# bridgedp/hunter_bipedal_control

Measured on NVIDIA H100. Metric: MPC+WBC control-step solves/sec (Hunter N=100), higher is better.
Workload: dtype f64

## Files before the change

hunter_bipedal_control_b200/csrc/hb_api.cu:

```cuda
#include <cuda_runtime.h>
#include <math.h>
#include <stdio.h>
#include <stdlib.h>
#include <string.h>

#include <new>

#include "../../include/hunter_b200.h"
#include "hb_common.cuh"
#include "hb_mpc.cuh"
#include "hb_planner.h"
#include <algorithm>
#include <string>
#include <utility>
#include <atomic>
#include <mutex>
#include <cstring>
#include <thread>
#include <vector>
#include "hb_qp.cuh"
#include "hb_rbd.cuh"
#include "hb_sqp.cuh"
#include "hb_wbc.cuh"
#include "hb_hoqp.cuh"
#include "hb_rollout.cuh"
#include "hb_estimator.cuh"
#include "hb_trajectory.cuh"
#include "hb_reference.cuh"

using namespace hb;

template <class T> struct InstanceSetting {
  T* dev;
  int n;
  std::vector<T> host;
  const T* get() const { return n > 0 ? dev : nullptr; }
};

struct hb_ctx {
  hb_config cfg;
  hb_wbc_settings wbc;
  int32_t wbc_form;
  int device;
  cudaStream_t stream;
  cudaStream_t stream_main, stream_aux;
  int base;
  int64_t launches;
  double *dxt, *dut, *perf;
  void* sqp_mem; double *lin, *proj, *rk;
  int32_t* flags;
  double *xdes, *udes;
  int32_t *wstatus, *witers, *wmode;
  void* hoqp_mem; double* hoqp_scratch;
  double *cyc_xref, *cyc_swing, *cyc_tk;
  int32_t *cyc_mode, *cyc_nn;
  double *res_t0, *res_xt, *res_ut, *res_tk;
  int32_t *res_mode, *res_nn;
  int res_valid;
  double* res_sol; int res_sol_valid;
  double* res_stance;
  void* ro_mem;
  hb_rollout_command* ro_cmd; hb_plan_input* ro_in; hb_reference* ro_refs; hb_solve_info* ro_info; int32_t* ro_pstat;
  double *ro_t0, *ro_x0, *ro_feet, *ro_sol, *ro_jcmd, *ro_jtau, *ro_tau, *ro_held, *ro_tnow, *ro_wrench;
  void* re_mem;
  double *re_quat, *re_gyro, *re_acc, *re_jpos, *re_jvel, *re_rbd;
  uint8_t* re_flag;
  InstanceSetting<hb_push_schedule> pushes;
  InstanceSetting<hb_plant_variation> variations;
  InstanceSetting<hb_terrain> terrains;
  void* arena; size_t arena_cap;
  void* pinned; size_t pinned_cap;
  int last_cuda;
  size_t last_h2d_bytes;
  int prof_on, prof_n;
  cudaEvent_t* prof_ev;
  int* prof_kind;
};

namespace {

enum { HB_OK = 0, HB_EINVAL = -1, HB_ECUDA = -2, HB_ENOMEM = -3, HB_ECAP = -4, HB_EPLAN = -5, HB_ECOMM = -6 };

#define CK(call)                                   \
  do {                                             \
    cudaError_t e__ = (call);                      \
    if (e__ != cudaSuccess) { if (ctx) ctx->last_cuda = (int)e__; return HB_ECUDA; } \
  } while (0)

constexpr int PROF_MAX = 4096;
enum { K_UNPROFILED = -1, K_BACKWARD = 0, K_FORWARD_LS = 1, K_WBC_ASSEMBLE = 2, K_QP = 3, K_OTHER = 4, K_LIN = 5, K_LQ = 6, K_NKINDS = 7 };

template <class T> cudaError_t dalloc(T** p, size_t n) { return cudaMalloc(reinterpret_cast<void**>(p), n * sizeof(T)); }

inline void prof_begin(hb_ctx* ctx, int kind) {
  if (ctx->prof_on && ctx->prof_n < PROF_MAX) { ctx->prof_kind[ctx->prof_n] = kind; cudaEventRecord(ctx->prof_ev[2 * ctx->prof_n], ctx->stream); }
}
inline void prof_end(hb_ctx* ctx) {
  if (ctx->prof_on && ctx->prof_n < PROF_MAX) { cudaEventRecord(ctx->prof_ev[2 * ctx->prof_n + 1], ctx->stream); ctx->prof_n++; }
}

template <class... P, class... A>
int launch(hb_ctx* ctx, int kind, void (*kernel)(P...), dim3 grid, dim3 block, size_t smem, A&&... args) {
  if (kind != K_UNPROFILED) prof_begin(ctx, kind);
  kernel<<<grid, block, smem, ctx->stream>>>(std::forward<A>(args)...);
  if (kind != K_UNPROFILED) prof_end(ctx);
  ctx->launches++;
  CK(cudaGetLastError());
  return HB_OK;
}

int set_device(hb_ctx* ctx) { return cudaSetDevice(ctx->device) == cudaSuccess ? HB_OK : HB_ECUDA; }

enum Cap : bool { UNCAPPED = false, CAPPED = true };
constexpr int EMPTY = 1;
inline bool no_host_check() { return true; }
template <class F = bool (*)()> int enter(hb_ctx* ctx, int B, bool args, Cap cap, const F& host_ok = no_host_check) {
  if (!ctx || B < 0 || !args) return HB_EINVAL;
  if (B == 0) return EMPTY;
  if (cap && ctx->base + B > ctx->cfg.max_batch) return HB_ECAP;
  if (!host_ok()) return HB_EINVAL;
  return set_device(ctx);
}
#define ENTER(...)                                                   \
  do {                                                               \
    const int rc__ = enter(__VA_ARGS__);                             \
    if (rc__) return rc__ == EMPTY ? HB_OK : rc__;                   \
  } while (0)

template <class T> bool all_ok(int B, const T* src, bool (*ok)(const T&)) {
  if (src) for (int i = 0; i < B; ++i) if (!ok(src[i])) return false;
  return true;
}
// ... 147 lines not shown
    case HB_ENOMEM: return "out of memory";
    case HB_ECAP: return "batch exceeds context capacity";
    case HB_EPLAN: return "reference planner: swing phase without take-off / touch-down time, or reference capacity exceeded";
    case HB_ECOMM: return "NCCL not available or a collective failed (hb_shard_last_error)";
    default: return "unknown error";
  }
}

int hb_create(const hb_config* cfg, int device, hb_ctx** out) {
  if (!cfg || !out || cfg->horizon_N < 1 || cfg->horizon_N > HB_MAX_HORIZON || cfg->max_batch < 1 || !(cfg->dt > 0.0) || cfg->time_horizon < 0.0) return HB_EINVAL;
  hb_ctx* ctx = new (std::nothrow) hb_ctx();
  if (!ctx) return HB_ENOMEM;
  memset(ctx, 0, sizeof(*ctx));
  ctx->cfg = *cfg;
  ctx->device = device;
  hb_default_wbc_settings(&ctx->wbc);
  if (cudaSetDevice(device) != cudaSuccess) { hb_destroy(ctx); return HB_ECUDA; }
  if (cudaStreamCreateWithFlags(&ctx->stream, cudaStreamNonBlocking) != cudaSuccess) { ctx->stream = nullptr; hb_destroy(ctx); return HB_ECUDA; }
  ctx->stream_main = ctx->stream;
  if (cudaStreamCreateWithFlags(&ctx->stream_aux, cudaStreamNonBlocking) != cudaSuccess) { ctx->stream_aux = nullptr; hb_destroy(ctx); return HB_ECUDA; }
  Model* m = new Model();
  memset(m, 0, sizeof(Model));
  for (int b = 0; b < NBODY; ++b) {
    for (int i = 0; i < 3; ++i) { m->joint_xyz[3 * b + i] = HB_JOINT_XYZ[3 * b + i]; m->com[3 * b + i] = HB_BODY_COM[3 * b + i]; }
    for (int i = 0; i < 9; ++i) m->inertia[9 * b + i] = HB_BODY_INERTIA[9 * b + i];
    m->mass[b] = HB_BODY_MASS[b];
    int code = 0;
    for (int i = 0; i < 3; ++i) if (HB_JOINT_AXIS[3 * b + i] != 0.0) code = (HB_JOINT_AXIS[3 * b + i] > 0 ? 1 : -1) * (i + 1);
    m->joint_axis[b] = code;
  }
  m->total_mass = HB_TOTAL_MASS;
  for (int i = 0; i < 12; ++i) m->contact_offset[i] = HB_CONTACT_OFFSET[i];
  for (int j = 0; j < NJ; ++j) { m->joint_lower[j] = HB_JOINT_LOWER[j]; m->joint_upper[j] = HB_JOINT_UPPER[j]; m->joint_vel_limit[j] = HB_JOINT_VEL_LIMIT[j]; m->torque_limit[j] = HB_WBC_TORQUE_LIMITS[j % 5]; }
  for (int i = 0; i < NX; ++i) m->Q[i] = HB_Q_DIAG[i];
  cudaError_t e = cudaMemcpyToSymbol(c_model, m, sizeof(Model));
  if (e == cudaSuccess) {
    double* dR = nullptr;
    e = dalloc(&dR, NU * NU);
    if (e == cudaSuccess) {
      init_input_cost_kernel<<<1, 32, 0, ctx->stream>>>(dR);
      e = cudaStreamSynchronize(ctx->stream);
      if (e == cudaSuccess) e = cudaMemcpy(m->R, dR, sizeof(double) * NU * NU, cudaMemcpyDeviceToHost);
      if (e == cudaSuccess) e = cudaMemcpyToSymbol(c_model, m, sizeof(Model));
      cudaFree(dR);
    }
  }
  if (e == cudaSuccess) {
    double tab[32 * LQ_LANE_TAB] = {};
    for (int l = 0; l < 32; ++l) {
      double* t = tab + l * LQ_LANE_TAB;
      if (l < NX) t[0] = m->Q[l];
      if (l < 12) t[1] = m->R[l * NU + l];
      if (l >= 12 && l < NU) for (int j = 0; j < NJ; ++j) t[2 + j] = m->R[l * NU + 12 + j];
      if (l < 10) { t[12] = m->joint_lower[l]; t[13] = m->joint_upper[l]; }
      else if (l < 20) { t[12] = -m->joint_vel_limit[l - 10]; t[13] = m->joint_vel_limit[l - 10]; }
    }
    e = cudaMemcpyToSymbol(g_lq_lane, tab, sizeof(tab));
  }
  delete m;
  if (e != cudaSuccess) { ctx->last_cuda = (int)e; hb_destroy(ctx); return HB_ECUDA; }
  const size_t B = cfg->max_batch, N = cfg->horizon_N;
  bool ok = true;
  ok = ok && dalloc(&ctx->dxt, B * (N + 1) * NX) == cudaSuccess && dalloc(&ctx->dut, B * N * NU) == cudaSuccess;
  ok = ok && dalloc(&ctx->perf, B * 4) == cudaSuccess && dalloc(&ctx->flags, B) == cudaSuccess;
  ok = ok && dalloc(&ctx->xdes, B * NX) == cudaSuccess && dalloc(&ctx->udes, B * NU) == cudaSuccess;
  ok = ok && dalloc(&ctx->wstatus, B) == cudaSuccess && dalloc(&ctx->witers, B) == cudaSuccess && dalloc(&ctx->wmode, B) == cudaSuccess;
  ok = ok && dalloc(&ctx->cyc_xref, B * (N + 1) * NX) == cudaSuccess && dalloc(&ctx->cyc_swing, B * (N + 1) * 24) == cudaSuccess;
  ok = ok && dalloc(&ctx->cyc_mode, B * (N + 1)) == cudaSuccess && dalloc(&ctx->cyc_tk, B * (N + 1)) == cudaSuccess && dalloc(&ctx->cyc_nn, B) == cudaSuccess;
  ok = ok && dalloc(&ctx->res_xt, B * (N + 1) * NX) == cudaSuccess && dalloc(&ctx->res_ut, B * N * NU) == cudaSuccess && dalloc(&ctx->res_t0, B) == cudaSuccess;
  ok = ok && dalloc(&ctx->res_mode, B * (N + 1)) == cudaSuccess && dalloc(&ctx->res_tk, B * (N + 1)) == cudaSuccess && dalloc(&ctx->res_nn, B) == cudaSuccess;
  ok = ok && dalloc(&ctx->res_sol, B * NWBC) == cudaSuccess && dalloc(&ctx->res_stance, B * 12) == cudaSuccess;
  if (!ok) { hb_destroy(ctx); return HB_ENOMEM; }
  {
    cudaError_t fe = cudaSuccess;
    auto attr = [&](const void* fn, size_t bytes) { if (fe == cudaSuccess) fe = cudaFuncSetAttribute(fn, cudaFuncAttributeMaxDynamicSharedMemorySize, (int)bytes); };
    attr((const void*)probe_flow_map_kernel, sizeof(ProbeShared));
    attr((const void*)qp_batch_kernel, 200 * 1024);
    attr((const void*)wbc_fused_kernel, wbc_fused_doubles() * sizeof(double));
    attr((const void*)hoqp_kernel, hoqp_smem_bytes());
    attr((const void*)hwbc_fused_kernel, hwbc_fused_bytes());
    attr((const void*)lin_kernel, 4 * sizeof(LinHalf) + sizeof(ChainModel));
    attr((const void*)lq_kernel, sizeof(LqShared));
    attr((const void*)riccati_kernel, sizeof(RicShared));
    attr((const void*)forward_linesearch2_kernel, sizeof(Fw2Shared));
    attr((const void*)warm_shift_kernel, sizeof(double) * ((N + 1) * NX + N * NU));
    for (const void* fn : {(const void*)wbc_fused_kernel, (const void*)riccati_kernel, (const void*)lq_kernel, (const void*)hwbc_fused_kernel})
      if (fe == cudaSuccess) fe = cudaFuncSetAttribute(fn, cudaFuncAttributePreferredSharedMemoryCarveout, (int)cudaSharedmemCarveoutMaxShared);
    if (fe != cudaSuccess) { ctx->last_cuda = (int)fe; hb_destroy(ctx); return HB_ECUDA; }
  }
  *out = ctx;
  return HB_OK;
}

int hb_destroy(hb_ctx* ctx) {
  if (!ctx) return HB_EINVAL;
  cudaSetDevice(ctx->device);
  void* ptrs[] = {ctx->sqp_mem, ctx->dxt, ctx->dut, ctx->perf, ctx->flags, ctx->xdes, ctx->udes, ctx->wstatus, ctx->witers, ctx->wmode,
                  ctx->hoqp_mem, ctx->cyc_xref, ctx->cyc_swing, ctx->cyc_tk, ctx->cyc_mode, ctx->cyc_nn, ctx->res_t0, ctx->res_xt,
                  ctx->res_ut, ctx->res_tk, ctx->res_mode, ctx->res_nn, ctx->res_sol, ctx->res_stance, ctx->arena, ctx->ro_mem, ctx->re_mem,
                  ctx->pushes.dev, ctx->variations.dev, ctx->terrains.dev};
  for (void* p : ptrs) if (p) cudaFree(p);
  if (ctx->pinned) cudaFreeHost(ctx->pinned);
  if (ctx->prof_ev) { for (int i = 0; i < 2 * PROF_MAX; ++i) cudaEventDestroy(ctx->prof_ev[i]); delete[] ctx->prof_ev; delete[] ctx->prof_kind; }
  if (ctx->stream_aux) cudaStreamDestroy(ctx->stream_aux);
  if (ctx->stream_main) cudaStreamDestroy(ctx->stream_main);
  else if (ctx->stream) cudaStreamDestroy(ctx->stream);
  delete ctx;
  return HB_OK;
}

int hb_sync(hb_ctx* ctx) {
  if (!ctx) return HB_EINVAL;
  CK(cudaStreamSynchronize(ctx->stream));
  return HB_OK;
}
int hb_profile_enable(hb_ctx* ctx, int on) {
  if (!ctx) return HB_EINVAL;
  if (set_device(ctx)) return HB_ECUDA;
  if (on && !ctx->prof_ev) {
    ctx->prof_ev = new (std::nothrow) cudaEvent_t[2 * PROF_MAX];
    ctx->prof_kind = new (std::nothrow) int[PROF_MAX];
    if (!ctx->prof_ev || !ctx->prof_kind) return HB_ENOMEM;
    for (int i = 0; i < 2 * PROF_MAX; ++i) CK(cudaEventCreate(&ctx->prof_ev[i]));
  }
  ctx->prof_on = on ? 1 : 0;
  ctx->prof_n = 0;
  return HB_OK;
}

int hb_profile_read(hb_ctx* ctx, double* ms_per_kind, int64_t* count_per_kind) {
  if (!ctx || !ms_per_kind || !count_per_kind) return HB_EINVAL;
  if (set_device(ctx)) return HB_ECUDA;
  CK(cudaStreamSynchronize(ctx->stream));
  for (int k = 0; k < K_NKINDS; ++k) { ms_per_kind[k] = 0.0; count_per_kind[k] = 0; }
  for (int i = 0; i < ctx->prof_n; ++i) {
    float ms = 0.f;
    CK(cudaEventElapsedTime(&ms, ctx->prof_ev[2 * i], ctx->prof_ev[2 * i + 1]));
    ms_per_kind[ctx->prof_kind[i]] += ms;
    count_per_kind[ctx->prof_kind[i]]++;
  }
  ctx->prof_n = 0;
  return HB_OK;
}

const char* hb_last_cuda_error(const hb_ctx* ctx) { return ctx ? cudaGetErrorString((cudaError_t)ctx->last_cuda) : "no context"; }

int64_t hb_launch_count(const hb_ctx* ctx) { return ctx ? ctx->launches : 0; }
int64_t hb_last_reference_upload_bytes(const hb_ctx* ctx) { return ctx ? (int64_t)ctx->last_h2d_bytes : 0; }
void* hb_stream(hb_ctx* ctx) { return ctx ? (void*)ctx->stream : nullptr; }

static int launch_qp(hb_ctx* ctx, int B, int n, int m, const double* H, const double* g, const double* A, const double* lbA, const double* ubA,
                     size_t sH, size_t sA, size_t sB, const int32_t* m_per, double* x, int32_t* status, int32_t* iters) {
  if (!qp_shape_ok(n, m)) return HB_EINVAL;
  const size_t per_warp = qp_workspace_doubles(n) * sizeof(double);
  int wpb = (int)((200 * 1024) / per_warp);
  if (wpb < 1) return HB_EINVAL;
  if (wpb > 1) wpb = 1;
  const int blocks = (B + wpb - 1) / wpb;
  return launch(ctx, K_QP, qp_batch_kernel, blocks, 32 * wpb, per_warp * wpb, B, n, m, H, g, A, lbA, ubA, sH, sA, sB, m_per, ctx->cfg.wbc_rho,
                ctx->cfg.qp_max_iter, x, status, iters);
}

int hb_wbc_qp_batch_dev(hb_ctx* ctx, int B, int n, int m, const double* H, const double* g, const double* A, const double* lbA,
                        const double* ubA, double* x, int32_t* status, int32_t* iters) {
  ENTER(ctx, B, H && g && A && lbA && ubA && x, UNCAPPED);
  return launch_qp(ctx, B, n, m, H, g, A, lbA, ubA, (size_t)n * n, (size_t)m * n, (size_t)m, nullptr, x, status, iters);
}

int hb_wbc_solve_batch_dev(hb_ctx* ctx, int B, const double* x_des, const double* u_des, const double* rbd, const int32_t* mode,
                           const uint8_t* stance_mode, double* sol, int32_t* status) {
  ENTER(ctx, B, x_des && u_des && rbd && mode && sol, CAPPED);
  return launch(ctx, K_QP, wbc_fused_kernel, B, 32, wbc_fused_doubles() * sizeof(double), B, ctx->wbc, x_des, u_des, rbd, mode, stance_mode,
                ctx->cfg.wbc_rho, ctx->cfg.qp_max_iter, sol, status ? status : ctx->wstatus + ctx->base, ctx->witers + ctx->base);
}

int hb_wbc_assemble_batch_dev(hb_ctx* ctx, int B, const double* x_des, const double* u_des, const double* rbd, const int32_t* mode,
                              const uint8_t* stance_mode, double* H, double* g, double* A, double* lbA, double* ubA, int32_t* m_rows) {
  ENTER(ctx, B, x_des && u_des && rbd && mode && H && g && A && lbA && ubA && m_rows, UNCAPPED);
  const int wpb = 4;
  return launch(ctx, K_WBC_ASSEMBLE, wbc_assemble_kernel, (B + wpb - 1) / wpb, 32 * wpb, sizeof(WbcShared) * wpb, B, ctx->wbc, x_des, u_des, rbd, mode,
                stance_mode, H, g, A, lbA, ubA, m_rows);
}

int hb_wbc_qp_rows_batch_dev(hb_ctx* ctx, int B, int n, int m_alloc, const int32_t* m_rows, const double* H, const double* g, const double* A,
                             const double* lbA, const double* ubA, double* x, int32_t* status, int32_t* iters) {
  ENTER(ctx, B, m_rows && H && g && A && lbA && ubA && x, UNCAPPED);
  return launch_qp(ctx, B, n, m_alloc, H, g, A, lbA, ubA, (size_t)n * n, (size_t)m_alloc * n, (size_t)m_alloc, m_rows, x, status, iters);
}

static int hoqp_reserve(hb_ctx* ctx) {
  const size_t Bc = ctx->cfg.max_batch;
  return reserve_group(&ctx->hoqp_mem, [&](void* m) {
    size_t off = 0;
    ctx->hoqp_scratch = carve<double>(m, off, Bc * HQ_SCRATCH);
    return off;
  });
}

int hb_hoqp_solve_batch_dev(hb_ctx* ctx, int B, const hb_hoqp_problem* problems, double* x, double* slack, int32_t* status) {
  ENTER(ctx, B, problems && x, CAPPED);
  const int rc = hoqp_reserve(ctx);
  if (rc) return rc;
  return launch(ctx, K_QP, hoqp_kernel, B, 32, hoqp_smem_bytes(), B, problems, ctx->hoqp_scratch, 2 * ctx->cfg.qp_max_iter, x, slack, status);
}

static int hwbc_tasks_dev(hb_ctx* ctx, int B, const double* x_des, const double* u_des, const double* rbd, const int32_t* mode, hb_hoqp_problem* problems) {
  return launch(ctx, K_WBC_ASSEMBLE, hwbc_tasks_kernel, B, 32, 0, B, ctx->wbc, x_des, u_des, rbd, mode, problems);
}

int hb_hierarchical_wbc_solve_batch_dev(hb_ctx* ctx, int B, const double* x_des, const double* u_des, const double* rbd, const int32_t* mode, double* sol,
                                        int32_t* status) {
  ENTER(ctx, B, x_des && u_des && rbd && mode && sol, CAPPED);
  return launch(ctx, K_QP, hwbc_fused_kernel, B, 32, hwbc_fused_bytes(), B, ctx->wbc, x_des, u_des, rbd, mode, 2 * ctx->cfg.qp_max_iter, sol, status);
}

static int controller_wbc_dev(hb_ctx* ctx, int B, const double* x_des, const double* u_des, const double* rbd, const int32_t* mode,
                              const uint8_t* stance_mode, double* sol, int32_t* status) {
  if (ctx->wbc_form == HB_WBC_HIERARCHICAL)
    return hb_hierarchical_wbc_solve_batch_dev(ctx, B, x_des, u_des, rbd, mode, sol, status ? status : ctx->wstatus + ctx->base);
  return hb_wbc_solve_batch_dev(ctx, B, x_des, u_des, rbd, mode, stance_mode, sol, status);
}

int hb_mpc_cold_start_batch_dev(hb_ctx* ctx, int B, const double* x0, const int32_t* mode, double* x_traj, double* u_traj) {
  ENTER(ctx, B, x0 && mode && x_traj && u_traj, UNCAPPED);
  return launch(ctx, K_UNPROFILED, cold_start_kernel, B, 128, 0, B, ctx->cfg.horizon_N, x0, mode, x_traj, u_traj);
}

static int mpc_solve_impl(hb_ctx* ctx, int B, const double* x0, const double* x_ref, const double* swing_ref, const int32_t* mode,
                          double* x_traj, double* u_traj, hb_solve_info* info, const double* tk, const int32_t* nn) {
  ENTER(ctx, B, x0 && x_ref && swing_ref && mode && x_traj && u_traj && (tk == nullptr) == (nn == nullptr), CAPPED);
  const size_t Bc = ctx->cfg.max_batch, Nc = ctx->cfg.horizon_N;
  int rc = reserve_group(&ctx->sqp_mem, [&](void* m) {
    size_t off = 0;
    ctx->lin = carve<double>(m, off, Bc * Nc * LIN_STRIDE); ctx->proj = carve<double>(m, off, Bc * Nc * PJ_STRIDE);
    ctx->rk = carve<double>(m, off, Bc * Nc * RK_STRIDE);
    return off;
  });
  if (rc) return rc;
  SqpArgs a;
  a.tk = tk; a.nn = nn;
  a.B = B; a.N = ctx->cfg.horizon_N; a.dt = ctx->cfg.dt; a.x_ref = x_ref; a.swing = swing_ref; a.mode = mode; a.xt = x_traj; a.ut = u_traj;
  {
    const size_t o = (size_t)ctx->base, Nn = (size_t)ctx->cfg.horizon_N;
    a.lin = ctx->lin + o * Nn * LIN_STRIDE; a.proj = ctx->proj + o * Nn * PJ_STRIDE; a.rk = ctx->rk + o * Nn * RK_STRIDE;
    a.dxt = ctx->dxt + o * (Nn + 1) * NX; a.dut = ctx->dut + o * Nn * NU; a.perf = ctx->perf + o * 4; a.flags = ctx->flags + o; a.x0 = x0;
  }
  const int N = a.N, NP = (N + 1) / 2;
  const long long nw = (long long)B * NP;
  rc = launch(ctx, K_LIN, lin_kernel, (unsigned)((nw + 1) / 2), 64, 4 * sizeof(LinHalf) + sizeof(ChainModel), a);
  if (!rc) rc = launch(ctx, K_LQ, lq_kernel, (unsigned)((long long)B * N), 32, sizeof(LqShared), a);
  if (!rc) rc = launch(ctx, K_BACKWARD, riccati_kernel, B, 64, sizeof(RicShared), a);
  if (!rc) rc = launch(ctx, K_FORWARD_LS, forward_linesearch2_kernel, B, 32, sizeof(Fw2Shared), a, ctx->cfg.line_search_max_trials, info);
  return rc;
}

int hb_mpc_solve_batch_dev(hb_ctx* ctx, int B, const double* x0, const double* x_ref, const double* swing_ref, const int32_t* mode,
                           double* x_traj, double* u_traj, hb_solve_info* info) {
  return mpc_solve_impl(ctx, B, x0, x_ref, swing_ref, mode, x_traj, u_traj, info, nullptr, nullptr);
}

int hb_mpc_solve_grid_batch_dev(hb_ctx* ctx, int B, const double* x0, const double* node_times, const int32_t* n_intervals, const double* x_ref,
                                const double* swing_ref, const int32_t* mode, double* x_traj, double* u_traj, hb_solve_info* info) {
  if (!node_times || !n_intervals) return HB_EINVAL;
  return mpc_solve_impl(ctx, B, x0, x_ref, swing_ref, mode, x_traj, u_traj, info, node_times, n_intervals);
}

static int policy_eval_impl(hb_ctx* ctx, int B, double t_rel, const double* x_traj, const double* u_traj, const int32_t* mode, double* x_des,
                            double* u_des, int32_t* mode_out, const double* tk, const int32_t* nn) {
  ENTER(ctx, B, x_traj && u_traj && mode && x_des && u_des && (tk == nullptr) == (nn == nullptr), UNCAPPED);
  const int wpb = 4;
  return launch(ctx, K_UNPROFILED, policy_eval_kernel, (B + wpb - 1) / wpb, 32 * wpb, 0, B, ctx->cfg.horizon_N, ctx->cfg.dt, t_rel, x_traj, u_traj, mode,
                x_des, u_des, mode_out, tk, nn, nullptr, nullptr);
}

int hb_policy_eval_batch_dev(hb_ctx* ctx, int B, double t_rel, const double* x_traj, const double* u_traj, const int32_t* mode, double* x_des,
                             double* u_des, int32_t* mode_out) {
  return policy_eval_impl(ctx, B, t_rel, x_traj, u_traj, mode, x_des, u_des, mode_out, nullptr, nullptr);
}

int hb_policy_eval_grid_batch_dev(hb_ctx* ctx, int B, double t_rel, const double* node_times, const int32_t* n_intervals, const double* x_traj,
                                  const double* u_traj, const int32_t* mode, double* x_des, double* u_des, int32_t* mode_out) {
  if (!node_times || !n_intervals) return HB_EINVAL;
  return policy_eval_impl(ctx, B, t_rel, x_traj, u_traj, mode, x_des, u_des, mode_out, node_times, n_intervals);
}

int hb_time_grid_batch_dev(hb_ctx* ctx, int B, const double* t0, const hb_reference* refs, double* node_times, int32_t* n_intervals, int32_t* status) {
  ENTER(ctx, B, t0 && refs && node_times && n_intervals, UNCAPPED);
  const double T = ctx->cfg.time_horizon > 0.0 ? ctx->cfg.time_horizon : ctx->cfg.horizon_N * ctx->cfg.dt;
  return launch(ctx, K_UNPROFILED, time_grid_kernel, (B + 127) / 128, 128, 0, B, ctx->cfg.horizon_N, ctx->cfg.dt, T, t0, refs, node_times, n_intervals, status);
}

static int control_step_impl(hb_ctx* ctx, int B, double t_rel, const double* x0, const double* x_ref, const double* swing_ref, const int32_t* mode,
                             const double* rbd, double* x_traj, double* u_traj, hb_solve_info* info, double* wbc_sol, double* torque,
                             int32_t* wbc_status, const double* tk, const int32_t* nn) {
  ENTER(ctx, B, x0 && x_ref && swing_ref && mode && rbd && x_traj && u_traj && wbc_sol && (tk == nullptr) == (nn == nullptr), CAPPED);
  int rc = mpc_solve_impl(ctx, B, x0, x_ref, swing_ref, mode, x_traj, u_traj, info, tk, nn);
  if (rc) return rc;
  double* xdes = ctx->xdes + (size_t)ctx->base * NX; double* udes = ctx->udes + (size_t)ctx->base * NU; int32_t* wmode = ctx->wmode + ctx->base;
  rc = policy_eval_impl(ctx, B, t_rel, x_traj, u_traj, mode, xdes, udes, wmode, tk, nn);
  if (rc) return rc;
  rc = controller_wbc_dev(ctx, B, xdes, udes, rbd, wmode, nullptr, wbc_sol, wbc_status);
  if (!rc && torque) rc = launch(ctx, K_UNPROFILED, torque_kernel, (B * NJ + 127) / 128, 128, 0, B, wbc_sol, torque);
  return rc;
}

int hb_control_step_batch_dev(hb_ctx* ctx, int B, double t_rel, const double* x0, const double* x_ref, const double* swing_ref, const int32_t* mode,
                              const double* rbd, double* x_traj, double* u_traj, hb_solve_info* info, double* wbc_sol, double* torque,
                              int32_t* wbc_status) {
  return control_step_impl(ctx, B, t_rel, x0, x_ref, swing_ref, mode, rbd, x_traj, u_traj, info, wbc_sol, torque, wbc_status, nullptr, nullptr);
}

static int wbc_fallback(hb_ctx* ctx, int B, bool no_prev, const int32_t* wbc_status, double* wbc_sol, double* torque) {
  if (!wbc_status) return HB_OK;
  const int have_prev = (!no_prev && ctx->res_sol_valid >= ctx->base + B) ? 1 : 0;
  const int rc = launch(ctx, K_UNPROFILED, wbc_fallback_kernel, (B * NWBC + 127) / 128, 128, 0, B, have_prev, wbc_status, wbc_sol,
                        ctx->res_sol + (size_t)ctx->base * NWBC, torque);
  if (rc) return rc;
  if (ctx->res_sol_valid < ctx->base + B) ctx->res_sol_valid = ctx->base + B;
  return HB_OK;
}

static int resident_cycle_impl(hb_ctx* ctx, int B, int cold_start, double t_rel, const double* t0, const double* x0, const hb_reference* refs,
                               const double* rbd, hb_solve_info* info, double* wbc_sol, double* torque, int32_t* wbc_status, bool run_wbc) {
  ENTER(ctx, B, t0 && x0 && refs && rbd, CAPPED, [&] { return cold_start || ctx->res_valid >= ctx->base + B; });
  const size_t N = ctx->cfg.horizon_N, o = (size_t)ctx->base;
  double* xref = ctx->cyc_xref + o * (N + 1) * NX; double* swing = ctx->cyc_swing + o * (N + 1) * 24; int32_t* mode = ctx->cyc_mode + o * (N + 1);
  double* xt = ctx->res_xt + o * (N + 1) * NX; double* ut = ctx->res_ut + o * N * NU; double* tres = ctx->res_t0 + o;
  const bool grid = ctx->cfg.event_nodes != 0;
  double* tk = grid ? ctx->cyc_tk + o * (N + 1) : nullptr; int32_t* nn = grid ? ctx->cyc_nn + o : nullptr;
  double* tkres = grid ? ctx->res_tk + o * (N + 1) : nullptr; int32_t* nnres = grid ? ctx->res_nn + o : nullptr;
  int rc = HB_OK;
  if (grid) {
    rc = hb_time_grid_batch_dev(ctx, B, t0, refs, tk, nn, nullptr);
    if (rc) return rc;
    rc = hb_reference_expand_grid_batch_dev(ctx, B, tk, refs, xref, swing, mode);
// ... 906 lines not shown
```

hunter_bipedal_control_b200/csrc/hb_sqp.cuh:

```cuda
#pragma once
#include "hb_common.cuh"
#include "hb_mpc.cuh"
#include "hb_rbd.cuh"

namespace hb {

constexpr int LIN_F1 = 0, LIN_F2 = 22, LIN_A1 = 44, LIN_A2 = 242, LIN_BF1 = 440, LIN_BF2 = 476, LIN_BV1 = 512, LIN_BV2 = 572,
              LIN_EPOS = 632, LIN_EVEL = 644, LIN_DPQ = 656, LIN_DVX = 812, LIN_DVV = 1076, LIN_STRIDE = 1200;
constexpr int NTMAX = 16;
constexpr int NVMAX = 8;
constexpr int PJ_BT = 0, PJ_AT = 144, PJ_PXV = 342, PJ_NV = 562, PJ_BTV = 642, PJ_QV = 664, PJ_RV = 686, PJ_META = 702, PJ_PEV = 710,
              PJ_QT = 720, PJ_PT = 1204, PJ_RF = 1380, PJ_RN = 1416, PJ_STRIDE = 1480;
constexpr int PJ_RT_PACKED = PJ_STRIDE - PJ_RF;
static_assert(PJ_AT + 9 * NX == PJ_PXV && PJ_RN + NVMAX * NVMAX == PJ_STRIDE && PJ_PEV + NJ == PJ_QT, "projected record blocks are contiguous");
static_assert(PJ_QT % 2 == 0 && PJ_PT % 2 == 0 && PJ_RF % 2 == 0 && PJ_STRIDE % 2 == 0, "bulk-copied blocks start on 16 bytes");
constexpr int RK_STRIDE = NTMAX * NX + NTMAX;

struct LinHalf {
  double x[NX], u[NU], x2[NX], f[NX];
  double Acm[6 * 16], Jc[12 * 16], dp[12 * NDIR], dv[12 * NDIR];
  double Abinv[36], AbinvAj[6 * NJ], vgen[16], epos[12], evel[12], com[3];
  double sn[NDIR], cs[NDIR];
  double dh[6 * NDIR], dcom[3 * NDIR], dvb[6 * NDIR];
  double vals[2 * 6];
// ... 1015 lines not shown
        for (int c = 0; c < NTP; ++c) { sh.kff[c] = -col[c]; rk[NTMAX * NX + c] = -col[c]; }
      }
    }
    __syncwarp();
    if (lane < NX) {
      double s0 = in.qt[lane], s1 = 0.0;
      if (lane == 1) s1 = s1 + sh.sb[1];
      else if (lane < 3) s0 = s0 + sh.sb[lane];
#pragma unroll
      for (int k = 3; k < NX; ++k) {
        if (k & 1) s1 = fma(in.At3[(k - 3) * NX + lane], sh.sb[k], s1);
        else s0 = fma(in.At3[(k - 3) * NX + lane], sh.sb[k], s0);
      }
#pragma unroll
      for (int c = 0; c < NTP; ++c) s0 = fma(sh.Hux[c * NX + lane], sh.kff[c], s0);
      sh.sv[lane] = s0 + s1;
    }
  } else {
    mbar_wait(&sh.bar[3], ph);
    __syncwarp();
    rowmm_by<NX, 1>(sh.S, NX, NX, [&](double (&c)[NX], int i) {
      acc_rows(c, [&](int k) { return (k == i) ? 1.0 : 0.0; }, sh.SA, NX, 3);
      acc_rows(c, [&](int k) { return in.At3[k * NX + i]; }, sh.SA + 3 * NX, NX, 19);
    });
  }
  __syncthreads();
  if (warp == 0) rowmm<12, true, 1>(sh.S, NX, sh.Hux, NX, K, NX, NX, NTP);
  else rowmm<10, true, 1>(sh.S + 12, NX, sh.Hux, NX, K + 12, NX, NX, NTP);
  __syncthreads();
  for (int t = threadIdx.x; t < NX * (NX - 1) / 2; t += 64) {
    const int d = t / NX + 1, i = t - (d - 1) * NX, j = (i + d) % NX;
    const double v = 0.5 * (sh.S[i * NX + j] + sh.S[j * NX + i]);
    sh.S[i * NX + j] = v; sh.S[j * NX + i] = v;
  }
  __syncthreads();
}

__global__ void __launch_bounds__(64) riccati_kernel(SqpArgs a) {
  extern __shared__ __align__(16) unsigned char smem_raw[];
  RicShared& sh = *reinterpret_cast<RicShared*>(smem_raw);
  const int inst = blockIdx.x, lane = threadIdx.x & 31, warp = threadIdx.x >> 5;
  const double* proj = a.proj + (size_t)inst * a.N * PJ_STRIDE;
  const int N = sqp_nn(a, inst);
  if (threadIdx.x == 0) { for (int b = 0; b < 4; ++b) mbar_init(&sh.bar[b], 1); }
  __syncthreads();
  if (warp == 1 && lane == 0) ric_prefetch_tma(sh.in[(N - 1) & 1], proj + (size_t)(N - 1) * PJ_STRIDE, &sh.bar[(N - 1) & 1]);
  unsigned ph_in0 = 0u, ph_in1 = 0u;
  for (int idx = threadIdx.x; idx < TS; idx += 64) sh.S[idx] = 0.0;
  if (threadIdx.x < NX) sh.sv[threadIdx.x] = 0.0;
  bool fail = false;
  double merit = 0.0, dyn = 0.0, eqs = 0.0;
  __syncthreads();
  for (int k = N - 1; k >= 0; --k) {
    const double* rec = proj + (size_t)k * PJ_STRIDE;
    double* rk = a.rk + ((size_t)inst * a.N + k) * RK_STRIDE;
    const unsigned ph = (unsigned)(N - 1 - k) & 1u;
    if (k & 1) { mbar_wait(&sh.bar[1], ph_in1); ph_in1 ^= 1u; } else { mbar_wait(&sh.bar[0], ph_in0); ph_in0 ^= 1u; }
    RicNodeIn& in = sh.in[k & 1];
    const int nt = (int)in.meta[0], nf = (int)in.meta[1], nv = (int)in.meta[2];
    if (warp == 0) {
      if (lane == 0) {
        fence_proxy_async();
        mbar_expect_tx(&sh.bar[2], (unsigned)((nv * NX + PJ_RT_PACKED) * sizeof(double)));
        if (nv > 0) bulk_g2s(sh.Hux + nf * NX, rec + PJ_PT, nv * NX * sizeof(double), &sh.bar[2]);
        bulk_g2s(sh.Huu + HUU_RP, rec + PJ_RF, PJ_RT_PACKED * sizeof(double), &sh.bar[2]);
      }
    } else if (k > 0 && lane == 0) {
      ric_prefetch_tma(sh.in[(k - 1) & 1], proj + (size_t)(k - 1) * PJ_STRIDE, &sh.bar[(k - 1) & 1]);
    }
    merit += in.meta[3]; dyn += in.meta[4]; eqs += in.meta[5];
    if (in.meta[6] != 0.0) fail = true;
    if (nf == 12 && nt == nt_regular(12)) riccati_node<12, 12>(sh, in, rec, rk, fail, warp, ph);
    else if (nf == 6 && nt == nt_regular(6)) riccati_node<10, 6>(sh, in, rec, rk, fail, warp, ph);
    else if (nf == 0 && nt == nt_regular(0)) riccati_node<6, 0>(sh, in, rec, rk, fail, warp, ph);
    else riccati_node<NTMAX, -1>(sh, in, rec, rk, fail, warp, ph);
  }
  if (threadIdx.x == 0) {
    double* pf = a.perf + (size_t)inst * 4;
    pf[0] = merit; pf[1] = dyn; pf[2] = eqs; pf[3] = 0.0;
    a.flags[inst] = fail ? 1 : 0;
  }
}

struct FwNode {
  double Bt9[9 * NTMAX], At9[9 * NX], Pxv[NJ * NX], Nv[NJ * NVMAX], bt[NX], qt[NX], rt[NTMAX], meta[8], pev[NJ];
  double K[NTMAX * NX], kff[NTMAX], u[NU];
};
static_assert(offsetof(FwNode, At9) == PJ_AT * sizeof(double) && offsetof(FwNode, pev) == PJ_PEV * sizeof(double) &&
              offsetof(FwNode, K) == PJ_QT * sizeof(double) && offsetof(FwNode, u) == offsetof(FwNode, K) + RK_STRIDE * sizeof(double),
              "FwNode mirrors the record and the gains");
struct Fw2Shared {
  FwNode nd[2];
  double dx[NX], dxn[NX], w[NTMAX];
  unsigned long long bar[2];
};
static_assert(sizeof(FwNode) % 16 == 0 && (NJ * sizeof(double)) % 16 == 0 && (NJ * NX * sizeof(double)) % 16 == 0, "bulk copies need 16-byte multiples");

__device__ __forceinline__ void fw_prefetch_tma(FwNode& n, const double* __restrict__ rec, const double* __restrict__ rk, const double* __restrict__ uk,
                                                unsigned long long* bar) {
  fence_proxy_async();
  mbar_expect_tx(bar, (unsigned)sizeof(FwNode));
  bulk_g2s(n.Bt9, rec, PJ_QT * sizeof(double), bar);
  bulk_g2s(n.K, rk, RK_STRIDE * sizeof(double), bar);
  bulk_g2s(n.u, uk, sizeof(n.u), bar);
}

__global__ void __launch_bounds__(32) forward_linesearch2_kernel(SqpArgs a, int max_trials, void* info_out) {
  extern __shared__ __align__(16) unsigned char smem_raw[];
  Fw2Shared& sh = *reinterpret_cast<Fw2Shared*>(smem_raw);
  const int inst = blockIdx.x, lane = threadIdx.x, NS = a.N;
  const int N = sqp_nn(a, inst);
  double* xt = a.xt + (size_t)inst * (NS + 1) * NX;
  double* ut = a.ut + (size_t)inst * NS * NU;
  double* dxt = a.dxt + (size_t)inst * (NS + 1) * NX;
  double* dut = a.dut + (size_t)inst * NS * NU;
  const double* xref = a.x_ref + (size_t)inst * (NS + 1) * NX;
  const double* swing = a.swing + (size_t)inst * (NS + 1) * 24;
  const int32_t* mode = a.mode + (size_t)inst * (NS + 1);
  const double* proj = a.proj + (size_t)inst * NS * PJ_STRIDE;
  const double* rkb = a.rk + (size_t)inst * NS * RK_STRIDE;
  if (lane == 0) { mbar_init(&sh.bar[0], 1); mbar_init(&sh.bar[1], 1); }
  __syncwarp();
  if (lane == 0) fw_prefetch_tma(sh.nd[0], proj, rkb, ut, &sh.bar[0]);
  unsigned fph0 = 0u, fph1 = 0u;
  if (lane < NX) { xt[lane] = a.x0[(size_t)inst * NX + lane]; sh.dx[lane] = 0.0; dxt[lane] = 0.0; }
  double armijo = 0.0;
  bool finite = (a.flags[inst] == 0);
  const double im_mass = 1.0 / c_model.total_mass;
  for (int k = 0; k < N; ++k) {
    if (k + 1 < N && lane == 0) fw_prefetch_tma(sh.nd[(k + 1) & 1], proj + (size_t)(k + 1) * PJ_STRIDE, rkb + (size_t)(k + 1) * RK_STRIDE, ut + (k + 1) * NU, &sh.bar[(k + 1) & 1]);
    if (k & 1) { mbar_wait(&sh.bar[1], fph1); fph1 ^= 1u; } else { mbar_wait(&sh.bar[0], fph0); fph0 ^= 1u; }
    const FwNode& nd = sh.nd[k & 1];
    const int nt = (int)nd.meta[0], nf = (int)nd.meta[1], nv = (int)nd.meta[2];
    const int md_k = mode[k];
    const double dtk = sqp_dt(a, inst, k);
    unsigned fmask = 0u;
#pragma unroll
    for (int c = 0; c < 4; ++c) if (contact_flag(md_k, c)) fmask |= 7u << (3 * c);
    double arm = 0.0;
    if (lane < nt) {
      double s = nd.kff[lane];
#pragma unroll
      for (int j = 0; j < NX; ++j) s = fma(nd.K[lane * NX + j], sh.dx[j], s);
      sh.w[lane] = s;
      arm = nd.rt[lane] * s;
    }
    __syncwarp();
    if (lane < NX) {
      double du;
      if (lane < 12) {
        if (contact_flag(md_k, lane / 3)) du = sh.w[__popc(fmask & ((1u << lane) - 1u))];
        else du = -nd.u[lane];
      } else {
        const int i = lane - 12;
        du = nd.pev[i];
#pragma unroll
        for (int j = 0; j < NX; ++j) du = fma(nd.Pxv[i * NX + j], sh.dx[j], du);
        for (int c = 0; c < nv; ++c) du = fma(nd.Nv[i * NVMAX + c], sh.w[nf + c], du);
      }
      double s = nd.bt[lane];
      if (lane >= 3 && lane < 12) {
        const double* ar = nd.At9 + (lane - 3) * NX;
        const double* br = nd.Bt9 + (lane - 3) * NTMAX;
        double s1 = 0.0;
#pragma unroll
        for (int j = 0; j < NX; j += 2) { s = fma(ar[j], sh.dx[j], s); s1 = fma(ar[j + 1], sh.dx[j + 1], s1); }
        s += s1;
        for (int c = 0; c < nt; ++c) s = fma(br[c], sh.w[c], s);
      } else if (lane < 3) {
        double fsum = 0.0;
#pragma unroll
        for (int c = 0; c < 4; ++c) if (contact_flag(md_k, c)) fsum += sh.w[__popc(fmask & ((1u << (3 * c + lane)) - 1u))];
        s += sh.dx[lane] + (dtk * im_mass) * fsum;
      } else {
        s += sh.dx[lane] + dtk * (du - nd.pev[lane - 12]);
      }
      sh.dxn[lane] = s;
      dxt[(k + 1) * NX + lane] = s;
      arm += nd.qt[lane] * sh.dx[lane];
      dut[k * NU + lane] = du;
      if (!isfinite(s) || !isfinite(du)) finite = false;
    }
    armijo += warp_sum(arm);
    __syncwarp();
    if (lane < NX) sh.dx[lane] = sh.dxn[lane];
    __syncwarp();
  }
  finite = __all_sync(HB_FULL_MASK, finite);
  const double* pf = a.perf + (size_t)inst * 4;
  const double merit0 = pf[0], v0 = sqrt(pf[1] + pf[2]);
  const double gamma_c = 1e-6, armijoFactor = 1e-4, alpha_decay = 0.5, alpha_min = 1e-4;
  double alpha = 1.0, merit1 = merit0, v1 = v0;
  bool accepted = false;
  int trials = 0;
  if (finite) {
    while (alpha >= alpha_min && trials < max_trials) {
      double ms = 0.0, ds = 0.0, es = 0.0;
      for (int k = lane; k < N; k += 32) {
        const double dt = sqp_dt(a, inst, k);
        double x[NX], u[NU], xn[NX], f1[NX], f2[NX], x2[NX], ep[12], ev[12], xr[NX], sw[24];
        for (int i = 0; i < NX; ++i) { x[i] = xt[k * NX + i] + alpha * dxt[k * NX + i]; xn[i] = xt[(k + 1) * NX + i] + alpha * dxt[(k + 1) * NX + i]; xr[i] = xref[k * NX + i]; }
        for (int i = 0; i < NU; ++i) u[i] = ut[k * NU + i] + alpha * dut[k * NU + i];
        for (int i = 0; i < 24; ++i) sw[i] = swing[k * 24 + i];
        flow_map_lane(x, u, f1, ep, ev);
        for (int i = 0; i < NX; ++i) x2[i] = x[i] + dt * f1[i];
        flow_map_lane(x2, u, f2, nullptr, nullptr);
        double d2 = 0.0;
        for (int i = 0; i < NX; ++i) { const double d = x[i] + 0.5 * dt * (f1[i] + f2[i]) - xn[i]; d2 += d * d; }
        double cost, e2;
        node_values_lane(x, u, xr, sw, mode[k], ep, ev, cost, e2);
        ms += dt * cost; ds += dt * d2; es += dt * e2;
      }
      ms = warp_sum(ms); ds = warp_sum(ds); es = warp_sum(es);
      ++trials;
      const double vn = sqrt(ds + es);
      const double am = alpha * armijo;
      bool acc;
      if (vn > HB_SQP_G_MAX) acc = vn < (1.0 - gamma_c) * v0;
      else if (vn < HB_SQP_G_MIN && v0 < HB_SQP_G_MIN && am < 0.0) acc = ms < merit0 + armijoFactor * am;
      else acc = ms < (merit0 - gamma_c * v0) || vn < (1.0 - gamma_c) * v0;
      if (isfinite(ms) && isfinite(vn) && acc) { accepted = true; merit1 = ms; v1 = vn; break; }
      alpha *= alpha_decay;
    }
  }
  if (accepted) {
    auto axpy = [&](double* y, const double* d, int n) {
      int idx = lane;
      for (; idx + 96 < n; idx += 128) {
        const double y0 = y[idx], y1 = y[idx + 32], y2 = y[idx + 64], y3 = y[idx + 96];
        const double d0 = d[idx], d1 = d[idx + 32], d2 = d[idx + 64], d3 = d[idx + 96];
        y[idx] = fma(alpha, d0, y0); y[idx + 32] = fma(alpha, d1, y1); y[idx + 64] = fma(alpha, d2, y2); y[idx + 96] = fma(alpha, d3, y3);
      }
      for (; idx < n; idx += 32) y[idx] = fma(alpha, d[idx], y[idx]);
    };
    axpy(xt, dxt, (N + 1) * NX);
    axpy(ut, dut, N * NU);
  }
  if (lane == 0 && info_out) {
    struct Info { double alpha, merit0, merit1, viol0, viol1, armijo; int32_t status, n_trials; };
    Info* io = reinterpret_cast<Info*>(info_out) + inst;
    io->alpha = accepted ? alpha : 0.0; io->merit0 = merit0; io->merit1 = merit1; io->viol0 = v0; io->viol1 = v1;
    io->armijo = armijo; io->status = finite ? 0 : 3; io->n_trials = trials;
  }
}

}
```

Measured before the change: 184,100.

## Split forward rollout and line search; evaluate first trial across all nodes in parallel

The fused forward-rollout plus line-search kernel becomes three kernels. A one-warp forward rollout stores the armijo term and finite flag, a node-parallel kernel evaluates the alpha=1 merit terms with one thread per node, and a one-warp accept kernel reuses those terms for the first trial, recomputing only for later trials. The TMA prefetch also copies only the active gain rows instead of the full gain block. This spreads the costly first-trial dynamics evaluation across many threads instead of 32 lanes per instance, at the cost of two extra launches and a global scratch buffer.

```diff
diff --git a/hunter_bipedal_control_b200/csrc/hb_api.cu b/hunter_bipedal_control_b200/csrc/hb_api.cu
--- a/hunter_bipedal_control_b200/csrc/hb_api.cu
+++ b/hunter_bipedal_control_b200/csrc/hb_api.cu
@@ -48,6 +48,7 @@
   int64_t launches;
   double *dxt, *dut, *perf;
   void* sqp_mem; double *lin, *proj, *rk;
+  double* ls_terms;
   int32_t* flags;
   double *xdes, *udes;
   int32_t *wstatus, *witers, *wmode;
@@ -361,7 +362,7 @@
     attr((const void*)lin_kernel, 4 * sizeof(LinHalf) + sizeof(ChainModel));
     attr((const void*)lq_kernel, sizeof(LqShared));
     attr((const void*)riccati_kernel, sizeof(RicShared));
-    attr((const void*)forward_linesearch2_kernel, sizeof(Fw2Shared));
+    attr((const void*)forward_kernel, sizeof(Fw2Shared));
     attr((const void*)warm_shift_kernel, sizeof(double) * ((N + 1) * NX + N * NU));
     for (const void* fn : {(const void*)wbc_fused_kernel, (const void*)riccati_kernel, (const void*)lq_kernel, (const void*)hwbc_fused_kernel})
       if (fe == cudaSuccess) fe = cudaFuncSetAttribute(fn, cudaFuncAttributePreferredSharedMemoryCarveout, (int)cudaSharedmemCarveoutMaxShared);
@@ -512,7 +513,7 @@
   int rc = reserve_group(&ctx->sqp_mem, [&](void* m) {
     size_t off = 0;
     ctx->lin = carve<double>(m, off, Bc * Nc * LIN_STRIDE); ctx->proj = carve<double>(m, off, Bc * Nc * PJ_STRIDE);
-    ctx->rk = carve<double>(m, off, Bc * Nc * RK_STRIDE);
+    ctx->rk = carve<double>(m, off, Bc * Nc * RK_STRIDE); ctx->ls_terms = carve<double>(m, off, Bc * Nc * 3);
     return off;
   });
   if (rc) return rc;
@@ -529,7 +530,11 @@
   rc = launch(ctx, K_LIN, lin_kernel, (unsigned)((nw + 1) / 2), 64, 4 * sizeof(LinHalf) + sizeof(ChainModel), a);
   if (!rc) rc = launch(ctx, K_LQ, lq_kernel, (unsigned)((long long)B * N), 32, sizeof(LqShared), a);
   if (!rc) rc = launch(ctx, K_BACKWARD, riccati_kernel, B, 64, sizeof(RicShared), a);
-  if (!rc) rc = launch(ctx, K_FORWARD_LS, forward_linesearch2_kernel, B, 32, sizeof(Fw2Shared), a, ctx->cfg.line_search_max_trials, info);
+  double* terms = ctx->ls_terms + (size_t)ctx->base * N * 3;
+  const long long nodes = (long long)B * N;
+  if (!rc) rc = launch(ctx, K_FORWARD_LS, forward_kernel, B, 32, sizeof(Fw2Shared), a);
+  if (!rc) rc = launch(ctx, K_FORWARD_LS, ls_trial_kernel, (unsigned)((nodes + LS_TRIAL_THREADS - 1) / LS_TRIAL_THREADS), LS_TRIAL_THREADS, 0, a, terms);
+  if (!rc) rc = launch(ctx, K_FORWARD_LS, ls_accept_kernel, B, 32, 0, a, terms, ctx->cfg.line_search_max_trials, info);
   return rc;
 }
 
diff --git a/hunter_bipedal_control_b200/csrc/hb_sqp.cuh b/hunter_bipedal_control_b200/csrc/hb_sqp.cuh
--- a/hunter_bipedal_control_b200/csrc/hb_sqp.cuh
+++ b/hunter_bipedal_control_b200/csrc/hb_sqp.cuh
@@ -1121,30 +1121,34 @@
   }
 }
 
+constexpr int LS_TRIAL_THREADS = 128;
 struct FwNode {
   double Bt9[9 * NTMAX], At9[9 * NX], Pxv[NJ * NX], Nv[NJ * NVMAX], bt[NX], qt[NX], rt[NTMAX], meta[8], pev[NJ];
   double K[NTMAX * NX], kff[NTMAX], u[NU];
 };
 static_assert(offsetof(FwNode, At9) == PJ_AT * sizeof(double) && offsetof(FwNode, pev) == PJ_PEV * sizeof(double) &&
-              offsetof(FwNode, K) == PJ_QT * sizeof(double) && offsetof(FwNode, u) == offsetof(FwNode, K) + RK_STRIDE * sizeof(double),
+              offsetof(FwNode, K) == PJ_QT * sizeof(double) && offsetof(FwNode, kff) == offsetof(FwNode, K) + NTMAX * NX * sizeof(double) &&
+              offsetof(FwNode, u) == offsetof(FwNode, K) + RK_STRIDE * sizeof(double),
               "FwNode mirrors the record and the gains");
 struct Fw2Shared {
   FwNode nd[2];
   double dx[NX], dxn[NX], w[NTMAX];
   unsigned long long bar[2];
 };
-static_assert(sizeof(FwNode) % 16 == 0 && (NJ * sizeof(double)) % 16 == 0 && (NJ * NX * sizeof(double)) % 16 == 0, "bulk copies need 16-byte multiples");
+static_assert(sizeof(FwNode) % 16 == 0 && (NX * sizeof(double)) % 16 == 0 && (NTMAX * sizeof(double)) % 16 == 0 && (NU * sizeof(double)) % 16 == 0,
+              "bulk copies need 16-byte multiples");
 
 __device__ __forceinline__ void fw_prefetch_tma(FwNode& n, const double* __restrict__ rec, const double* __restrict__ rk, const double* __restrict__ uk,
-                                                unsigned long long* bar) {
+                                                int nt, unsigned long long* bar) {
   fence_proxy_async();
-  mbar_expect_tx(bar, (unsigned)sizeof(FwNode));
+  mbar_expect_tx(bar, (unsigned)((PJ_QT + nt * NX + NTMAX + NU) * sizeof(double)));
   bulk_g2s(n.Bt9, rec, PJ_QT * sizeof(double), bar);
-  bulk_g2s(n.K, rk, RK_STRIDE * sizeof(double), bar);
+  if (nt > 0) bulk_g2s(n.K, rk, nt * NX * sizeof(double), bar);
+  bulk_g2s(n.kff, rk + NTMAX * NX, NTMAX * sizeof(double), bar);
   bulk_g2s(n.u, uk, sizeof(n.u), bar);
 }
 
-__global__ void __launch_bounds__(32) forward_linesearch2_kernel(SqpArgs a, int max_trials, void* info_out) {
+__global__ void __launch_bounds__(32) forward_kernel(SqpArgs a) {
   extern __shared__ __align__(16) unsigned char smem_raw[];
   Fw2Shared& sh = *reinterpret_cast<Fw2Shared*>(smem_raw);
   const int inst = blockIdx.x, lane = threadIdx.x, NS = a.N;
@@ -1153,21 +1157,27 @@
   double* ut = a.ut + (size_t)inst * NS * NU;
   double* dxt = a.dxt + (size_t)inst * (NS + 1) * NX;
   double* dut = a.dut + (size_t)inst * NS * NU;
-  const double* xref = a.x_ref + (size_t)inst * (NS + 1) * NX;
-  const double* swing = a.swing + (size_t)inst * (NS + 1) * 24;
   const int32_t* mode = a.mode + (size_t)inst * (NS + 1);
   const double* proj = a.proj + (size_t)inst * NS * PJ_STRIDE;
   const double* rkb = a.rk + (size_t)inst * NS * RK_STRIDE;
+  auto gain_rows = [&](int j) { const int r = (int)proj[(size_t)j * PJ_STRIDE + PJ_META]; return r < 0 ? 0 : (r > NTMAX ? NTMAX : r); };
+  int nt_next = 0;
   if (lane == 0) { mbar_init(&sh.bar[0], 1); mbar_init(&sh.bar[1], 1); }
   __syncwarp();
-  if (lane == 0) fw_prefetch_tma(sh.nd[0], proj, rkb, ut, &sh.bar[0]);
+  if (lane == 0) {
+    fw_prefetch_tma(sh.nd[0], proj, rkb, ut, gain_rows(0), &sh.bar[0]);
+    if (N > 1) nt_next = gain_rows(1);
+  }
   unsigned fph0 = 0u, fph1 = 0u;
   if (lane < NX) { xt[lane] = a.x0[(size_t)inst * NX + lane]; sh.dx[lane] = 0.0; dxt[lane] = 0.0; }
   double armijo = 0.0;
   bool finite = (a.flags[inst] == 0);
   const double im_mass = 1.0 / c_model.total_mass;
   for (int k = 0; k < N; ++k) {
-    if (k + 1 < N && lane == 0) fw_prefetch_tma(sh.nd[(k + 1) & 1], proj + (size_t)(k + 1) * PJ_STRIDE, rkb + (size_t)(k + 1) * RK_STRIDE, ut + (k + 1) * NU, &sh.bar[(k + 1) & 1]);
+    if (k + 1 < N && lane == 0) {
+      fw_prefetch_tma(sh.nd[(k + 1) & 1], proj + (size_t)(k + 1) * PJ_STRIDE, rkb + (size_t)(k + 1) * RK_STRIDE, ut + (k + 1) * NU, nt_next, &sh.bar[(k + 1) & 1]);
+      if (k + 2 < N) nt_next = gain_rows(k + 2);
+    }
     if (k & 1) { mbar_wait(&sh.bar[1], fph1); fph1 ^= 1u; } else { mbar_wait(&sh.bar[0], fph0); fph0 ^= 1u; }
     const FwNode& nd = sh.nd[k & 1];
     const int nt = (int)nd.meta[0], nf = (int)nd.meta[1], nv = (int)nd.meta[2];
@@ -1226,7 +1236,58 @@
     __syncwarp();
   }
   finite = __all_sync(HB_FULL_MASK, finite);
+  if (lane == 0) { a.perf[(size_t)inst * 4 + 3] = armijo; a.flags[inst] = finite ? 0 : 1; }
+}
+
+__device__ __forceinline__ void ls_node_terms(const SqpArgs& a, int inst, int k, double alpha, double& cost, double& d2, double& e2) {
+  const int NS = a.N;
+  const double* xt = a.xt + (size_t)inst * (NS + 1) * NX;
+  const double* ut = a.ut + (size_t)inst * NS * NU;
+  const double* dxt = a.dxt + (size_t)inst * (NS + 1) * NX;
+  const double* dut = a.dut + (size_t)inst * NS * NU;
+  const double* xref = a.x_ref + (size_t)inst * (NS + 1) * NX;
+  const double* swing = a.swing + (size_t)inst * (NS + 1) * 24;
+  const int32_t* mode = a.mode + (size_t)inst * (NS + 1);
+  const double dt = sqp_dt(a, inst, k);
+  double x[NX], u[NU], f1[NX], f2[NX], x2[NX];
+  for (int i = 0; i < NX; ++i) x[i] = xt[k * NX + i] + alpha * dxt[k * NX + i];
+  for (int i = 0; i < NU; ++i) u[i] = ut[k * NU + i] + alpha * dut[k * NU + i];
+  {
+    double ep[12], ev[12];
+    flow_map_lane(x, u, f1, ep, ev);
+    node_values_lane(x, u, xref + k * NX, swing + k * 24, mode[k], ep, ev, cost, e2);
+  }
+  for (int i = 0; i < NX; ++i) x2[i] = x[i] + dt * f1[i];
+  flow_map_lane(x2, u, f2, nullptr, nullptr);
+  d2 = 0.0;
+  for (int i = 0; i < NX; ++i) {
+    const double xn = xt[(k + 1) * NX + i] + alpha * dxt[(k + 1) * NX + i];
+    const double d = x[i] + 0.5 * dt * (f1[i] + f2[i]) - xn;
+    d2 += d * d;
+  }
+}
+
+__global__ void __launch_bounds__(LS_TRIAL_THREADS) ls_trial_kernel(SqpArgs a, double* __restrict__ terms) {
+  const long long t = (long long)blockIdx.x * LS_TRIAL_THREADS + threadIdx.x;
+  if (t >= (long long)a.B * a.N) return;
+  const int inst = (int)(t / a.N), k = (int)(t - (long long)inst * a.N);
+  if (k >= sqp_nn(a, inst) || a.flags[inst] != 0) return;
+  double cost, d2, e2;
+  ls_node_terms(a, inst, k, 1.0, cost, d2, e2);
+  double* o = terms + (size_t)t * 3;
+  o[0] = cost; o[1] = d2; o[2] = e2;
+}
+
+__global__ void __launch_bounds__(32) ls_accept_kernel(SqpArgs a, const double* __restrict__ terms, int max_trials, void* info_out) {
+  const int inst = blockIdx.x, lane = threadIdx.x, NS = a.N;
+  const int N = sqp_nn(a, inst);
+  double* xt = a.xt + (size_t)inst * (NS + 1) * NX;
+  double* ut = a.ut + (size_t)inst * NS * NU;
+  const double* dxt = a.dxt + (size_t)inst * (NS + 1) * NX;
+  const double* dut = a.dut + (size_t)inst * NS * NU;
   const double* pf = a.perf + (size_t)inst * 4;
+  const bool finite = (a.flags[inst] == 0);
+  const double armijo = pf[3];
   const double merit0 = pf[0], v0 = sqrt(pf[1] + pf[2]);
   const double gamma_c = 1e-6, armijoFactor = 1e-4, alpha_decay = 0.5, alpha_min = 1e-4;
   double alpha = 1.0, merit1 = merit0, v1 = v0;
@@ -1237,17 +1298,13 @@
       double ms = 0.0, ds = 0.0, es = 0.0;
       for (int k = lane; k < N; k += 32) {
         const double dt = sqp_dt(a, inst, k);
-        double x[NX], u[NU], xn[NX], f1[NX], f2[NX], x2[NX], ep[12], ev[12], xr[NX], sw[24];
-        for (int i = 0; i < NX; ++i) { x[i] = xt[k * NX + i] + alpha * dxt[k * NX + i]; xn[i] = xt[(k + 1) * NX + i] + alpha * dxt[(k + 1) * NX + i]; xr[i] = xref[k * NX + i]; }
-        for (int i = 0; i < NU; ++i) u[i] = ut[k * NU + i] + alpha * dut[k * NU + i];
-        for (int i = 0; i < 24; ++i) sw[i] = swing[k * 24 + i];
-        flow_map_lane(x, u, f1, ep, ev);
-        for (int i = 0; i < NX; ++i) x2[i] = x[i] + dt * f1[i];
-        flow_map_lane(x2, u, f2, nullptr, nullptr);
-        double d2 = 0.0;
-        for (int i = 0; i < NX; ++i) { const double d = x[i] + 0.5 * dt * (f1[i] + f2[i]) - xn[i]; d2 += d * d; }
-        double cost, e2;
-        node_values_lane(x, u, xr, sw, mode[k], ep, ev, cost, e2);
+        double cost, d2, e2;
+        if (trials == 0) {
+          const double* t = terms + ((size_t)inst * NS + k) * 3;
+          cost = t[0]; d2 = t[1]; e2 = t[2];
+        } else {
+          ls_node_terms(a, inst, k, alpha, cost, d2, e2);
+        }
         ms += dt * cost; ds += dt * d2; es += dt * e2;
       }
       ms = warp_sum(ms); ds = warp_sum(ds); es = warp_sum(es);
```

Result: no change. 185,900 (median of 6 runs) (+1.0%).
